# lupoglaz/DeepLocalProteinDocking

Hardware: AMD Instinct MI355X
Metric: pose correlations/sec (48ch x 64^3 pair, 6-degree SOI-sized generated rotation set) (higher is better)
Workload: dtype f32

## Files before the change

### deeplocalproteindocking_amd/csrc/dlpd_corr.hip

```cpp
#include <dlpd_platform.h>
#include "dlpd_fft.h"
#include "dlpd_internal.h"
#include "dlpd_trilinear.h"
#include "dlpd_k1.h"
#include "dlpd_k3.h"

#ifndef DLPD_K1CL_PAD
#define DLPD_K1CL_PAD 13
#endif
#ifndef DLPD_K1CL_PXOR
#define DLPD_K1CL_PXOR 0
#endif
#define DLPD_K1_UNROLL 2
DLPD_D float trilinear_fetch_quads(const float4* __restrict__ q, int L, float px, float py, float pz) {
  const float fx = floorf(px), fy = floorf(py), fz = floorf(pz);
  const int ix = (int)fx, iy = (int)fy, iz = (int)fz;
  const float ax = px - fx, ay = py - fy, az = pz - fz;
  const int hi = L - 1;
  const bool x0 = (ix >= 0) & (ix <= hi), x1 = (ix + 1 >= 0) & (ix + 1 <= hi);
  const bool y0 = (iy >= 0) & (iy <= hi), y1 = (iy + 1 >= 0) & (iy + 1 <= hi);
  const bool z0 = (iz >= 0) & (iz <= hi), z1 = (iz + 1 >= 0) & (iz + 1 <= hi);
  const float wx0 = x0 ? 1.f - ax : 0.f, wx1 = x1 ? ax : 0.f;
  const float wy0 = y0 ? 1.f - ay : 0.f, wy1 = y1 ? ay : 0.f;
  const float wz0 = z0 ? 1.f - az : 0.f, wz1 = z1 ? az : 0.f;
  const int cx0 = min(max(ix, 0), hi), cx1 = min(max(ix + 1, 0), hi);
  const int yb = min(max(iy, 0), hi - 1), zb = min(max(iz, 0), hi - 1);
  const int dy = iy - yb, dz = iz - zb;
  const int Q = L - 1;
  const float4 qa = q[((size_t)cx0 * Q + yb) * Q + zb];
  const float4 qb = q[((size_t)cx1 * Q + yb) * Q + zb];
  const float a_y0z0 = dy > 0 ? qa.z : qa.x, a_y0z1 = dy > 0 ? qa.w : qa.y;
  const float a_y1z0 = dy < 0 ? qa.x : qa.z, a_y1z1 = dy < 0 ? qa.y : qa.w;
  const float b_y0z0 = dy > 0 ? qb.z : qb.x, b_y0z1 = dy > 0 ? qb.w : qb.y;
  const float b_y1z0 = dy < 0 ? qb.x : qb.z, b_y1z1 = dy < 0 ? qb.y : qb.w;
  const float v000 = dz > 0 ? a_y0z1 : a_y0z0, v001 = dz < 0 ? a_y0z0 : a_y0z1;
  const float v010 = dz > 0 ? a_y1z1 : a_y1z0, v011 = dz < 0 ? a_y1z0 : a_y1z1;
  const float v100 = dz > 0 ? b_y0z1 : b_y0z0, v101 = dz < 0 ? b_y0z0 : b_y0z1;
  const float v110 = dz > 0 ? b_y1z1 : b_y1z0, v111 = dz < 0 ? b_y1z0 : b_y1z1;
  float acc = v000 * (wx0 * wy0 * wz0);
  acc += v001 * (wx0 * wy0 * wz1);
  acc += v010 * (wx0 * wy1 * wz0);
  acc += v011 * (wx0 * wy1 * wz1);
  acc += v100 * (wx1 * wy0 * wz0);
  acc += v101 * (wx1 * wy0 * wz1);
  acc += v110 * (wx1 * wy1 * wz0);
  acc += v111 * (wx1 * wy1 * wz1);
  return acc;
}

__global__ void __launch_bounds__(256) k_make_quads(const float* __restrict__ v, float4* __restrict__ q, int nvol, int L) {
  const int Q = L - 1;
  const size_t total = (size_t)nvol * L * Q * Q;
  for (size_t i = (size_t)blockIdx.x * blockDim.x + threadIdx.x; i < total; i += (size_t)gridDim.x * blockDim.x) {
    const int z = (int)(i % Q), y = (int)((i / Q) % Q);
    const size_t xv = i / ((size_t)Q * Q);
    const float* p = v + (xv * L + y) * L + z;
    q[i] = make_float4(p[0], p[1], p[L], p[L + 1]);
  }
}

__global__ void __launch_bounds__(256) k_rotate(const float* __restrict__ vol, const float* __restrict__ R,
                                                float* __restrict__ out, int B, int C, int L,
                                                long long vol_bstride, float c0) {
  const size_t L3 = (size_t)L * L * L;
  const size_t total = (size_t)B * C * L3;
  for (size_t i = (size_t)blockIdx.x * blockDim.x + threadIdx.x; i < total; i += (size_t)gridDim.x * blockDim.x) {
    const int z = (int)(i % L), y = (int)((i / L) % L), x = (int)((i / ((size_t)L * L)) % L);
    const int c = (int)((i / L3) % C), b = (int)(i / (L3 * C));
    const float* r = R + (size_t)b * 9;
    const float dx = x - c0, dy = y - c0, dz = z - c0;
    const float px = c0 + (r[0] * dx + r[3] * dy + r[6] * dz);
    const float py = c0 + (r[1] * dx + r[4] * dy + r[7] * dz);
    const float pz = c0 + (r[2] * dx + r[5] * dy + r[8] * dz);
    out[i] = trilinear_fetch(vol + (size_t)b * vol_bstride + (size_t)c * L3, L, px, py, pz);
  }
}

#ifdef DLPD_STAMPS
__device__ unsigned long long dlpd_stamps_k1[16];
extern "C" int dlpd_debug_read_stamps_k1(unsigned long long* host16) {
  if (hipMemcpyFromSymbol(host16, HIP_SYMBOL(dlpd_stamps_k1), 16 * sizeof(unsigned long long)) != hipSuccess) return 1;
  unsigned long long z[16] = {0};
  return hipMemcpyToSymbol(HIP_SYMBOL(dlpd_stamps_k1), z, sizeof(z)) == hipSuccess ? 0 : 1;
}
#endif
template <int N> __global__ void __launch_bounds__((N / 4) * FftPlan<N>::T)
k_rotate_zfft(const float* __restrict__ vol, const float* __restrict__ R, cplx* __restrict__ A,
              int CT, int nb, long long vol_bstride, int do_rotate, float c0, int CT_out, int c_base,
              int transposed, const float4* __restrict__ quads, int ext, const unsigned char* __restrict__ occ, int skip_empty) {
  constexpr int L = N / 2, NZ = N / 2 + 1, RS = N + 1, NP = L / 2;
  constexpr int T = FftPlan<N>::T, R1 = FftPlan<N>::R1, R2 = FftPlan<N>::R2;
  constexpr int NT = NP * T;
  __shared__ cplx S[NP * RS + N];
  cplx* tw = S + NP * RS;
  const int tid = threadIdx.x;
  const int bid = blockIdx.x, jj = bid >> 3;
  const int grp = (bid & 7) + 8 * (jj / L);
  if (grp >= CT * nb) return;
  const int c = grp % CT, b = grp / CT;
  if (do_rotate || !occ) init_twiddles<N>(tw, tid, NT);
  const int tr_flag = transposed;
  const int lane = tid & 63, wave = tid >> 6;
  (void)lane; (void)wave;
  DLPD_STAMP_DECL;
  const int x = jj % L;
  bool pencil_live = true;
  {
  const float* v = vol + (size_t)b * vol_bstride + (size_t)c * L * L * L;
  float* Sf = reinterpret_cast<float*>(S);
  if (do_rotate) {
    const float* r = R + (size_t)b * 9;
    const float r0 = r[tr_flag ? 3 : 0], r1 = r[tr_flag ? 4 : 1], r2 = r[tr_flag ? 5 : 2];
    const float r3 = r[tr_flag ? 0 : 3], r4 = r[tr_flag ? 1 : 4], r5 = r[tr_flag ? 2 : 5];
    const float r6 = r[6], r7 = r[7], r8 = r[8];
    const float dx = x - c0;
#pragma unroll DLPD_K1_UNROLL
    for (int s = tid; s < L * L; s += NT) {
      constexpr int TZ = 8, TYY = 64 / TZ;
      const int chunk = s >> 6, q = s & 63;
      const int y = (chunk / (L / TZ)) * TYY + q / TZ, z = (chunk % (L / TZ)) * TZ + q % TZ;
      const float dy = y - c0, dz = z - c0;
      const float px = c0 + (r0 * dx + r3 * dy + r6 * dz);
      const float py = c0 + (r1 * dx + r4 * dy + r7 * dz);
      const float pz = c0 + (r2 * dx + r5 * dy + r8 * dz);
      Sf[((y >> 1) * RS + z) * 2 + (y & 1)] =
          (max(x, max(y, z)) >= ext) ? 0.f
          : quads ? trilinear_fetch_quads(quads + (size_t)c * L * (L - 1) * (L - 1), L, px, py, pz)
                  : trilinear_fetch(v, L, px, py, pz);
    }
  } else {
    constexpr int NC = (L + 3) / 4;
    const unsigned char* ob = occ ? occ + ((size_t)b * NC + (x >> 2)) * NC * NC : nullptr;
    __shared__ unsigned char ocell[NC * NC];
    __shared__ int occ_any, yany[NC];
    if (ob) {
      if (tid == 0) occ_any = 0;
      if (tid < NC) yany[tid] = 0;
      __syncthreads();
      for (int i = tid; i < NC * NC; i += NT) {
        const unsigned char o = ob[i];
        ocell[i] = o;
        if (o) { occ_any = 1; yany[i / NC] = 1; }
      }
      __syncthreads();
      if (!occ_any) {
        if (skip_empty) return;
        cplx* a = A + ((size_t)b * CT_out + c_base + c) * NZ * L * L + (size_t)x * L;
        for (int s = tid; s < NP * NZ; s += NT)
          DLPD_STORE_STREAM(reinterpret_cast<float4*>(a + (size_t)(s / NP) * L * L + 2 * (s % NP)), make_float4(0.f, 0.f, 0.f, 0.f));
        return;
      }
      init_twiddles<N>(tw, tid, NT);
    }
    for (int s = tid; s < L * L; s += NT) {
      const int y = s / L, z = s % L;
      const bool zero = ob && !ocell[(y >> 2) * NC + (z >> 2)];
      Sf[((y >> 1) * RS + z) * 2 + (y & 1)] = zero ? 0.f : (tr_flag ? v[((size_t)y * L + x) * L + z] : v[((size_t)x * L + y) * L + z]);
    }
    pencil_live = !(ob && skip_empty) || yany[(tid % NP) >> 1];
  }
  DLPD_STAMP(0);
  __syncthreads();
  DLPD_STAMP(1);
  const int p = tid % NP, t = tid / NP;
  {
    FftPass<N, R1, 1, -1, T, L> ps;
    if (pencil_live) ps.load(S + p * RS, 1, t, tw);
    __syncthreads();
    if (pencil_live) ps.store(S + p * RS, 1, t);
    __syncthreads();
  }
  {
    FftPass<N, R2, R1, -1, T> ps;
    if (pencil_live) ps.load(S + p * RS, 1, t, tw);
    __syncthreads();
    if (pencil_live) ps.store(S + p * RS, 1, t);
    __syncthreads();
  }
  DLPD_STAMP(2);
  cplx* a = A + ((size_t)b * CT_out + c_base + c) * NZ * L * L + (size_t)x * L;
  for (int s = tid; s < NP * NZ; s += NT) {
    const int m = s % NP, k = s / NP;
    if (!pencil_live) continue;
    const cplx zk = S[m * RS + k];
    const cplx zn = S[m * RS + ((N - k) % N)];
    float4 o;
    o.x = 0.5f * (zk.x + zn.x);
    o.y = 0.5f * (zk.y - zn.y);
    o.z = 0.5f * (zk.y + zn.y);
    o.w = 0.5f * (zn.x - zk.x);
    DLPD_STORE_STREAM(reinterpret_cast<float4*>(a + (size_t)k * L * L + 2 * m), o);
  }
  DLPD_STAMP(3);
  }
  DLPD_STAMP_FLUSH(dlpd_stamps_k1, DLPD_STAMPS);
}

template <int N, bool OCC> __global__ void __launch_bounds__(K1ClCfg<N>::NP * FftPlan<N>::T)
k_rotate_zfft_cl(const float4* __restrict__ cl, const float* __restrict__ R, cplx* __restrict__ A,
                 int C, int nchunk, int vstride, int cstride, int nb, float c0, int CT_out, int c_base, int ext,
                 const unsigned char* __restrict__ occ, int skip_empty) {
  constexpr int L = N / 2, NZ = N / 2 + 1, NP = K1ClCfg<N>::NP, CC = K1ClCfg<N>::CC, YG = K1ClCfg<N>::YG, NPR = YG / 2;
  constexpr int LPV = CC / 4, SKEW = 16 / LPV;
  static_assert(CC * NPR == NP && L % YG == 0 && (NP * FftPlan<N>::T) % 64 == 0, "whole waves of pencils per block");
  constexpr int RS = N + DLPD_K1CL_PAD;
  constexpr int T = FftPlan<N>::T, R1 = FftPlan<N>::R1, R2 = FftPlan<N>::R2;
  constexpr int NT = NP * T;
  DLPD_DYN_SHARED(cplx, S);
  cplx* tw = S + NP * RS;
  const int tid = threadIdx.x;
  const int per = (L / YG) * nchunk;
  const int groups = nb * L, gper = (groups + 7) / 8;
  const int bid = blockIdx.x, seq = bid >> 3;
  const int g = (bid & 7) * gper + seq / per;
  if (seq / per >= gper || g >= groups) return;
#ifdef DLPD_K1_CHUNK_OUTER
  const int inner = seq % per, chunk = inner / (L / YG), yg = inner % (L / YG);
#else
  const int inner = seq % per, yg = inner / nchunk, chunk = inner % nchunk;
#endif
  const int b = g / L, x = g % L;
  constexpr int NC = (L + 3) / 4, YC = YG / 4;
  static_assert(YG % 4 == 0, "a block's rows are whole cells");
  __shared__ unsigned char occ_s[OCC ? YC * NC : 1];
  __shared__ int occ_any;
  if (OCC) {
    const unsigned char* ob = occ + (((size_t)b * NC + (x >> 2)) * NC + (yg * YG >> 2)) * NC;
    if (tid == 0) occ_any = 0;
    __syncthreads();
    if (tid < YC * NC) {
      const unsigned char o = ob[tid];
      occ_s[tid] = o;
      if (o) occ_any = 1;
    }
    __syncthreads();
    if (!occ_any) {
      if (skip_empty) return;
      for (int s = tid; s < NP * NZ; s += NT) {
        const int pm = s % NP, k = s / NP;
        const int c = chunk * CC + pm / NPR, m = pm % NPR;
        if (c < C)
          DLPD_STORE_STREAM(reinterpret_cast<float4*>(A + (((size_t)b * CT_out + c_base + c) * NZ + k) * L * L + (size_t)x * L +
                                                      yg * YG + 2 * m), make_float4(0.f, 0.f, 0.f, 0.f));
      }
      return;
    }
  }
  init_twiddles<N>(tw, tid, NT);
  {
    const K1ClRot rot = k1cl_load_rotation(R + (size_t)b * 9);
    for (int task = tid; task < NPR * L * LPV; task += NT) {
      const int q = task % LPV, z = (task / LPV) % L, m = (task / LPV) / L;
      const float4* src = cl + (size_t)chunk * cstride + q;
      float4 acc[2];
      if (OCC && !occ_s[((2 * m) >> 2) * NC + (z >> 2)])
        acc[0] = acc[1] = make_float4(0.f, 0.f, 0.f, 0.f);
      else
        k1cl_sample_rows(src, vstride, L, ext, c0, rot, x, yg * YG + 2 * m, z, acc);
      cplx* P = S + ((4 * q) * NPR + m) * RS + SKEW * q + z;
      P[0] = c_make(acc[0].x, acc[1].x);
      P[NPR * RS] = c_make(acc[0].y, acc[1].y);
      P[2 * NPR * RS] = c_make(acc[0].z, acc[1].z);
      P[3 * NPR * RS] = c_make(acc[0].w, acc[1].w);
    }
  }
  __syncthreads();
  const int p = (tid % NP) ^ DLPD_K1CL_PXOR, t = tid / NP;
  cplx* Sp = S + p * RS + SKEW * (p / (4 * NPR));
  {
    FftPass<N, R1, 1, -1, T, L> ps;
    ps.load(Sp, 1, t, tw);
    __syncthreads();
    ps.store(Sp, 1, t);
    __syncthreads();
  }
  {
    FftPass<N, R2, R1, -1, T> ps;
    ps.load(Sp, 1, t, tw);
    __syncthreads();
    ps.store(Sp, 1, t);
    __syncthreads();
  }
  for (int s = tid; s < NP * NZ; s += NT) {
    const int pm = s % NP, k = s / NP;
    const int c = chunk * CC + pm / NPR, m = pm % NPR;
    if (c < C) {
      const cplx* Z = S + pm * RS + SKEW * (pm / (4 * NPR));
      const cplx zk = Z[k];
      const cplx zn = Z[(N - k) % N];
      float4 o;
      o.x = 0.5f * (zk.x + zn.x);
      o.y = 0.5f * (zk.y - zn.y);
      o.z = 0.5f * (zk.y + zn.y);
      o.w = 0.5f * (zn.x - zk.x);
      cplx* a = A + (((size_t)b * CT_out + c_base + c) * NZ + k) * L * L + (size_t)x * L + yg * YG + 2 * m;
      DLPD_STORE_STREAM(reinterpret_cast<float4*>(a), o);
    }
  }
}

__global__ void __launch_bounds__(256) k_make_channels_last(const float* __restrict__ v, float4* __restrict__ cl, int C, int Cq, int L) {
  const size_t L3 = (size_t)L * L * L, total = L3 * Cq;
  for (size_t i = (size_t)blockIdx.x * blockDim.x + threadIdx.x; i < total; i += (size_t)gridDim.x * blockDim.x) {
    const int c4 = (int)(i % Cq);
    const size_t vox = i / Cq;
    float e[4];
#pragma unroll
    for (int j = 0; j < 4; j++) e[j] = (4 * c4 + j < C) ? v[(size_t)(4 * c4 + j) * L3 + vox] : 0.f;
    cl[i] = make_float4(e[0], e[1], e[2], e[3]);
  }
}

__global__ void __launch_bounds__(256) k_make_channel_chunks(const float* __restrict__ v, float4* __restrict__ out, int C, int CCq,
                                                             int nchunk, int L) {
  const size_t L3 = (size_t)L * L * L, total = L3 * CCq * nchunk;
  for (size_t i = (size_t)blockIdx.x * blockDim.x + threadIdx.x; i < total; i += (size_t)gridDim.x * blockDim.x) {
    const int q = (int)(i % CCq);
    const size_t vox = (i / CCq) % L3;
    const int c0 = 4 * ((int)(i / (CCq * L3)) * CCq + q);
    float e[4];
#pragma unroll
    for (int j = 0; j < 4; j++) e[j] = (c0 + j < C) ? v[(size_t)(c0 + j) * L3 + vox] : 0.f;
    out[i] = make_float4(e[0], e[1], e[2], e[3]);
  }
}

template <int N> static int launch_k1_cl(const float4* cl, const float* R, cplx* A, int C, int nb, float c0, hipStream_t st,
                                         int CT_out, int c_base, int ext = 0, const unsigned char* occ = nullptr, int skip_empty = 0,
                                         bool chunk_major = false) {
  constexpr int L = N / 2, RS = N + DLPD_K1CL_PAD, CCq = K1ClCfg<N>::CC / 4;
  const int Cq = ((C + DLPD_K1CL_CC - 1) / DLPD_K1CL_CC) * (DLPD_K1CL_CC / 4);
  const int nchunk = chunk_major ? (C + 4 * CCq - 1) / (4 * CCq) : Cq / CCq;
  const int vstride = chunk_major ? CCq : Cq, cstride = chunk_major ? L * L * L * CCq : CCq;
  const size_t shmem = (size_t)(K1ClCfg<N>::NP * RS + N) * sizeof(cplx);
  const int per = (L / K1ClCfg<N>::YG) * nchunk;
  const int gper = (nb * L + 7) / 8;
  dim3 grid((unsigned)(8 * gper * per)), block(K1ClCfg<N>::NP * FftPlan<N>::T);
  const int e = (ext > 0 && ext < L) ? ext : L;
  if (occ) {
    int rc = dlpd_set_max_dyn_shared((const void*)k_rotate_zfft_cl<N, true>, shmem);
    if (rc) return rc;
    DLPD_LAUNCH((k_rotate_zfft_cl<N, true>), grid, block, shmem, st, cl, R, A, C, nchunk, vstride, cstride, nb, c0, CT_out,
                c_base, e, occ, skip_empty);
  } else {
    int rc = dlpd_set_max_dyn_shared((const void*)k_rotate_zfft_cl<N, false>, shmem);
    if (rc) return rc;
    DLPD_LAUNCH((k_rotate_zfft_cl<N, false>), grid, block, shmem, st, cl, R, A, C, nchunk, vstride, cstride, nb, c0, CT_out,
                c_base, e, occ, 0);
  }
  return dlpd_check_launch();
}

__global__ void __launch_bounds__(256) k_rotated_occupancy(const unsigned char* __restrict__ occ_src, const float* __restrict__ R,
                                                           unsigned char* __restrict__ occ_out, int nb, int L, float c0) {
  const int nc = (L + 3) / 4, nc3 = nc * nc * nc;
  for (int i = blockIdx.x * blockDim.x + threadIdx.x; i < nb * nc3; i += gridDim.x * blockDim.x) {
    const int b = i / nc3, cell = i % nc3, cz = cell % nc, cy = (cell / nc) % nc, cx = cell / (nc * nc);
    const float* r = R + (size_t)b * 9;
    const float hx = 0.5f * (min(4 * cx + 3, L - 1) - 4 * cx), hy = 0.5f * (min(4 * cy + 3, L - 1) - 4 * cy),
                hz = 0.5f * (min(4 * cz + 3, L - 1) - 4 * cz);
    const float dx = 4 * cx + hx - c0, dy = 4 * cy + hy - c0, dz = 4 * cz + hz - c0;
    bool any = false;
    int lo[3], hi[3];
#pragma unroll
    for (int a = 0; a < 3; a++) {
      const float s = c0 + (r[a] * dx + r[3 + a] * dy + r[6 + a] * dz);
      const float e = fabsf(r[a]) * hx + fabsf(r[3 + a]) * hy + fabsf(r[6 + a]) * hz + 1e-3f * (1.f + fabsf(s));
      lo[a] = max((int)floorf(s - e), 0) >> 2;
      hi[a] = min((int)floorf(s + e) + 1, L - 1) >> 2;
    }
    for (int sx = lo[0]; sx <= hi[0]; sx++)
      for (int sy = lo[1]; sy <= hi[1]; sy++)
        for (int sz = lo[2]; sz <= hi[2]; sz++) any |= occ_src[(sx * nc + sy) * nc + sz] != 0;
    occ_out[i] = any ? 1 : 0;
  }
}
__global__ void __launch_bounds__(256) k_pencil_bits(const unsigned char* __restrict__ occ, unsigned* __restrict__ bits, int nb, int nc) {
  const int lane = threadIdx.x & 63, i = (blockIdx.x * blockDim.x + threadIdx.x) >> 6;
  bool any = false;
  if (i < nb * nc && lane < nc) {
    const unsigned char* o = occ + ((size_t)i * nc + lane) * nc;
    for (int cz = 0; cz < nc; cz++) any |= o[cz] != 0;
  }
  const unsigned long long m = __ballot(any);
  if (i < nb * nc && lane == 0) bits[i] = (unsigned)m;
}

template <int N, int MODE> struct K3Cfg { static constexpr int NT = 512, WC = 8, TY = 16; };
#ifndef DLPD_K3_80_NT
#define DLPD_K3_80_NT 640
#endif
template <int MODE> struct K3Cfg<80, MODE> { static constexpr int NT = (MODE == 0 ? 320 : DLPD_K3_80_NT), WC = 5, TY = 16; };
template <> struct K3Cfg<160, 0> { static constexpr int NT = 320, WC = 5, TY = 16; };
#ifndef DLPD_K3_160_NT
#define DLPD_K3_160_NT 640
#endif
template <> struct K3Cfg<160, 1> { static constexpr int NT = DLPD_K3_160_NT, WC = 5, TY = 8; };
template <> struct K3Cfg<160, 2> { static constexpr int NT = DLPD_K3_160_NT, WC = 5, TY = 8; };
#ifndef DLPD_K3_LAUNDER_160
#define DLPD_K3_LAUNDER_160 1
#endif
#ifdef DLPD_STAMPS
__device__ unsigned long long dlpd_stamps[16];
#endif
template <int N, int HP, int MODE> __global__ void __launch_bounds__((K3Cfg<N, MODE>::NT))
k_zifft_filter(const cplx* __restrict__ Bw, float* __restrict__ out, int CT, int C, int has_clash, int G,
               const float* __restrict__ W1t, const float* __restrict__ b1, const float* __restrict__ W2,
               float b2, int has_clip, float clip, float thr, K3Aux aux, K3Cand cd) {
  typedef K3Cfg<N, MODE> Cfg;
  typedef K3Lds<N, Cfg> Geo;
  constexpr int NZ = Geo::NZ, RS = Geo::RS, TY = Cfg::TY, NPAIR = Geo::NPAIR;
  constexpr int NT = Cfg::NT, WC = Cfg::WC;
  constexpr int CPW = Geo::CPW;
  constexpr int LPK = Geo::LPK;
  static_assert((NPAIR == 8 || NPAIR == 4) && WC * 64 <= NT, "one wave = 8 pencils x 8 threads");
  constexpr int EPT = (NPAIR * N) / NT > 0 ? (NPAIR * N) / NT : 1;
  constexpr int MSTEP = NT / N;
  static_assert((NPAIR * N) % NT == 0 || NPAIR * N < NT, "tile/thread mismatch");
  constexpr int RAWC = Geo::RAWC;
  DLPD_DYN_SHARED(cplx, S);
  cplx* tw = S + WC * 8 * RS;
  float4* raw = reinterpret_cast<float4*>(tw + N);
  const int tid = threadIdx.x, lane = tid & 63, wave = tid >> 6;
  const int y0 = blockIdx.x * TY, xo = blockIdx.y, b = blockIdx.z;

  constexpr int HPH = HP;
  float nrm[EPT * 2];
  float total[EPT * 2];
#pragma unroll
  for (int e = 0; e < EPT * 2; e++) { nrm[e] = 0.f; total[e] = b2; }
  const unsigned cand_tau = (MODE == 1 && cd.keys) ? *cd.tau : 0u;
  if (MODE == 1 && cd.keys && !cand_tau && tid == 0) cd.count[cd.nb + blockIdx.z] = 1u;
  const int zz = tid % N, m0 = tid / N;
  const bool owner = (NPAIR * N >= NT) || (m0 < NPAIR);
  const int tr = lane & 7, qr = lane >> 3;
  float4* rawg = raw + wave * CPW * RAWC;

  constexpr int NFULL = (N / 2) / LPK;
  static_assert(NZ * NPAIR == NFULL * 64 + NPAIR, "raw channel = NFULL full DMA instructions + one short one");
  auto issue_channel = [&](int cb) {
#pragma unroll
    for (int j = 0; j < CPW; j++) {
      const int g = wave * CPW + j;
      if (g < G && cb + g < CT) {
        const cplx* src = Bw + (((size_t)b * CT + cb + g) * NZ * N + xo) * N + y0;
        const cplx* lane_src = src + (size_t)(lane / NPAIR) * N * N + 2 * (lane % NPAIR);
        float4* rj = rawg + j * RAWC;
#pragma unroll
        for (int it = 0; it < NFULL; it++) DLPD_GLDS16(lane_src + (size_t)it * LPK * N * N, rj + it * 64);
        const int mt = lane % NPAIR;
        DLPD_GLDS16(src + (size_t)(N / 2) * N * N + 2 * mt, rj + NFULL * 64);
      }
    }
  };
  DLPD_STAMP_DECL;
  issue_channel(0);
  init_twiddles<N>(tw, tid, NT);
  constexpr int j0 = 0;
  float h[EPT * 2][HPH > 0 ? HPH : 1];
  if (MODE >= 1) {
    if (MODE == 1 && aux.C > 0 && aux.is_preact) {
      const int Na = aux.N;
      const size_t cstride = (size_t)Na * Na * Na;
      const float* ab = aux.p + (size_t)b * HP * cstride + ((size_t)(xo >> 1) * Na + (y0 >> 1)) * Na + (zz >> 1);
      if (owner) {
#pragma unroll
        for (int e = 0; e < EPT; e++)
#pragma unroll
          for (int j = 0; j < HP; j++) {
            const float v = ab[(size_t)j * cstride + (size_t)(m0 + e * MSTEP) * Na];
            h[2 * e][j] = v;
            h[2 * e + 1][j] = v;
          }
      }
    } else {
#pragma unroll
      for (int e = 0; e < EPT * 2; e++)
#pragma unroll
        for (int j = 0; j < HPH; j++) h[e][j] = b1[j0 + j];
    }
  }
  __syncthreads();

  for (int cbase = 0; cbase < CT; cbase += G) {
    const int gn = (CT - cbase) < G ? (CT - cbase) : G;
    if (wave * CPW < gn) {
      DLPD_WAIT_VMEM();
      DLPD_WAVE_SYNC();
      DLPD_STAMP(0);
#pragma unroll
      for (int j = 0; j < CPW; j++) {
        if (wave * CPW + j >= gn) break;
        int m, kq, lq = lane;
        if (N == 160 && DLPD_K3_LAUNDER_160) DLPD_OPAQUE(lq);
        if (NPAIR == 8) {
          m = (lq & 3) | (((lq >> 4) & 1) << 2);
          kq = ((lq >> 2) & 1) | (((lq >> 5) & 1) << 1) | (((lq >> 3) & 1) << 2);
        } else {
          m = lq % NPAIR;
          kq = lq / NPAIR;
        }
        const int rot = (NPAIR == 8) ? 2 * m : 0;
        const int slot = NPAIR * kq + m;
        cplx* P = S + (wave * 8 + j * NPAIR + m) * RS;
        const float4* rj = rawg + j * RAWC;
        constexpr int PCH = NFULL > 8 ? NFULL / 2 : NFULL;
        const float4 qh = rj[NFULL * 64 + (lane % NPAIR)];
#pragma unroll
        for (int it0 = 0; it0 < NFULL; it0 += PCH) {
          float4 q[PCH];
          int kk[PCH];
#pragma unroll
          for (int u = 0; u < PCH; u++) {
            const int it = (it0 + u + rot) % NFULL;
            kk[u] = it * LPK + kq;
            q[u] = rj[it * 64 + slot];
          }
#pragma unroll
          for (int u = 0; u < PCH; u++) {
            const int k = kk[u];
            const cplx lo = (k == 0) ? c_make(q[u].x, q[u].z) : c_make(q[u].x - q[u].w, q[u].y + q[u].z);
            const cplx hi = (k == 0) ? c_make(q[u].x, q[u].z) : c_make(q[u].x + q[u].w, q[u].z - q[u].y);
            P[pencil_in_pos<N>(k)] = lo;
            P[pencil_in_pos<N>((N - k) & (k == 0 ? 0 : ~0))] = hi;
          }
        }
        if (lane / NPAIR == 0) S[(wave * 8 + j * NPAIR + lane % NPAIR) * RS + pencil_in_pos<N>(N / 2)] = c_make(qh.x, qh.z);
      }
      DLPD_WAIT_LDS();
      DLPD_WAVE_SYNC();
    }
    DLPD_STAMP(1);
    issue_channel(cbase + G);
    DLPD_STAMP(2);
    if (wave * CPW < gn) {
      int tq = tr, qq = qr;
      if (N == 160 && DLPD_K3_LAUNDER_160) { DLPD_OPAQUE(tq); DLPD_OPAQUE(qq); }
      fft_wave_pencils<N, +1>(S, wave * 8, RS, qq, tq, tw);
    }
    DLPD_STAMP(3);
    DLPD_LDS_BARRIER();
    DLPD_STAMP(4);
    if (owner) {
      if (MODE == 0) {
        for (int g = 0; g < gn; g++) {
          const int c = cbase + g;
#pragma unroll
          for (int e = 0; e < EPT; e++) {
            const int m = m0 + e * MSTEP;
            const cplx val = S[(g * NPAIR + m) * RS + pencil_out_pos<N>(zz)];
            float v0 = val.x, v1 = val.y;
            if (has_clip && c < C) { v0 = DLPD_CLAMP(v0, clip); v1 = DLPD_CLAMP(v1, clip); }
            float* o = out + ((((size_t)b * CT + c) * N + xo) * N + y0 + 2 * m) * N + zz;
            o[0] = v0;
            o[N] = v1;
          }
        }
      } else {
        const int gs = (cbase + gn <= C) ? gn : (C - cbase > 0 ? C - cbase : 0);
        float wcur[HPH > 0 ? HPH : 1], wnxt[HPH > 0 ? HPH : 1];
        cplx vcur[EPT], vnxt[EPT];
        if (gs > 0) {
#pragma unroll
          for (int j = 0; j < HPH; j++) wcur[j] = W1t[(size_t)cbase * HP + j0 + j];
#pragma unroll
          for (int e = 0; e < EPT; e++) vcur[e] = S[(m0 + e * MSTEP) * RS + pencil_out_pos<N>(zz)];
        }
        for (int g = 0; g < gs; g++) {
          const int gn1 = (g + 1 < gs ? g + 1 : g);
#pragma unroll
          for (int j = 0; j < HPH; j++) wnxt[j] = W1t[(size_t)(cbase + gn1) * HP + j0 + j];
#pragma unroll
          for (int e = 0; e < EPT; e++) vnxt[e] = S[(gn1 * NPAIR + m0 + e * MSTEP) * RS + pencil_out_pos<N>(zz)];
          DLPD_SCHED_FENCE();
#pragma unroll
          for (int e = 0; e < EPT; e++) {
            float v0 = vcur[e].x, v1 = vcur[e].y;
            if (has_clip) { v0 = DLPD_CLAMP(v0, clip); v1 = DLPD_CLAMP(v1, clip); }
#pragma unroll
            for (int j = 0; j < HPH; j++) {
              h[2 * e][j] = fmaf(wcur[j], v0, h[2 * e][j]);
              h[2 * e + 1][j] = fmaf(wcur[j], v1, h[2 * e + 1][j]);
            }
          }
          DLPD_SCHED_FENCE();
#pragma unroll
          for (int j = 0; j < HPH; j++) wcur[j] = wnxt[j];
#pragma unroll
          for (int e = 0; e < EPT; e++) vcur[e] = vnxt[e];
        }
        if (has_clash && cbase + gn > C) {
          const int g = C - cbase;
#pragma unroll
          for (int e = 0; e < EPT; e++) {
            const cplx v = S[(g * NPAIR + m0 + e * MSTEP) * RS + pencil_out_pos<N>(zz)];
            nrm[2 * e] = v.x;
            nrm[2 * e + 1] = v.y;
          }
        }
      }
    }
    DLPD_STAMP(5);
    DLPD_LDS_BARRIER();
    DLPD_STAMP(6);
  }
  DLPD_STAMP_FLUSH(dlpd_stamps, DLPD_STAMPS);
  if (MODE == 1 && owner && aux.C > 0 && !aux.is_preact) {
    const int Na = aux.N;
    const float* ab = aux.p + (size_t)b * aux.C * Na * Na * Na + ((size_t)(xo >> 1) * Na + (y0 >> 1)) * Na + (zz >> 1);
    constexpr int CH = EPT > 2 ? 4 : 8;
    const size_t cstride = (size_t)Na * Na * Na;
    for (int cb = 0; cb < aux.C; cb += CH) {
      float av[CH][EPT];
#pragma unroll
      for (int k = 0; k < CH; k++)
#pragma unroll
        for (int e = 0; e < EPT; e++)
          av[k][e] = (cb + k < aux.C) ? ab[(size_t)(cb + k) * cstride + (size_t)(m0 + e * MSTEP) * Na] : 0.f;
#pragma unroll
      for (int k = 0; k < CH; k++) {
        if (cb + k < aux.C) {
          const float* w = W1t + (size_t)(C + cb + k) * HP + j0;
#pragma unroll
          for (int e = 0; e < EPT; e++) {
            const float v = av[k][e];
#pragma unroll
            for (int j = 0; j < HPH; j++) {
              h[2 * e][j] = fmaf(w[j], v, h[2 * e][j]);
              h[2 * e + 1][j] = fmaf(w[j], v, h[2 * e + 1][j]);
            }
          }
        }
      }
    }
  }
  if (MODE == 1 && owner) {
#pragma unroll
    for (int e = 0; e < EPT * 2; e++)
#pragma unroll
      for (int j = 0; j < HPH; j++) total[e] = fmaf(W2[j0 + j], fmaxf(h[e][j], 0.f), total[e]);
  }
// ... 655 lines not shown
```

### deeplocalproteindocking_amd/csrc/dlpd_k1.h

```cpp
#pragma once
#include <dlpd_platform.h>
#include "dlpd_fft.h"

#define DLPD_K1CL_CC 16
#ifndef DLPD_K1_YG160
#define DLPD_K1_YG160 8
#endif
#ifndef DLPD_K1_CC160
#define DLPD_K1_CC160 16
#endif
#ifndef DLPD_K1_YG128
#define DLPD_K1_YG128 16
#endif
template <int N> struct K1ClCfg {
  static constexpr int YG = (N == 128) ? DLPD_K1_YG128 : (N == 160 ? DLPD_K1_YG160 : 8), CC = (N == 160) ? DLPD_K1_CC160 : 128 / YG;
  static constexpr int NP = CC * (YG / 2);
};
struct K1ClRot { float r0, r1, r2, r3, r4, r5, r6, r7, r8; };
DLPD_D K1ClRot k1cl_load_rotation(const float* r) {
  K1ClRot o = {r[0], r[1], r[2], r[3], r[4], r[5], r[6], r[7], r[8]};
  return o;
}

DLPD_D void k1cl_sample_rows(const float4* __restrict__ src, int Cq, int L, int ext, float c0, const K1ClRot& r, int x, int yrow,
                             int z, float4 (&acc)[2]) {
  const float dx = x - c0, dz = z - c0;
  const int hi = L - 1;
#pragma unroll
      for (int u = 0; u < 2; u++) {
        const bool live = max(x, max(yrow + u, z)) < ext;
        const float dy = (yrow + u) - c0;
        const float px = c0 + (r.r0 * dx + r.r3 * dy + r.r6 * dz);
        const float py = c0 + (r.r1 * dx + r.r4 * dy + r.r7 * dz);
        const float pz = c0 + (r.r2 * dx + r.r5 * dy + r.r8 * dz);
        const float fx = floorf(px), fy = floorf(py), fz = floorf(pz);
        const int ix = (int)fx, iy = (int)fy, iz = (int)fz;
        const float ax = px - fx, ay = py - fy, az = pz - fz;
        const bool x0 = live & (ix >= 0) & (ix <= hi), x1 = live & (ix + 1 >= 0) & (ix + 1 <= hi);
        const bool y0 = (iy >= 0) & (iy <= hi), y1 = (iy + 1 >= 0) & (iy + 1 <= hi);
        const bool z0 = (iz >= 0) & (iz <= hi), z1 = (iz + 1 >= 0) & (iz + 1 <= hi);
        const float wx0 = x0 ? 1.f - ax : 0.f, wx1 = x1 ? ax : 0.f;
        const float wy0 = y0 ? 1.f - ay : 0.f, wy1 = y1 ? ay : 0.f;
        const float wz0 = z0 ? 1.f - az : 0.f, wz1 = z1 ? az : 0.f;
        const int cx0 = min(max(ix, 0), hi), cx1 = min(max(ix + 1, 0), hi);
        const int cy0 = min(max(iy, 0), hi), cy1 = min(max(iy + 1, 0), hi);
        const int cz0 = min(max(iz, 0), hi), cz1 = min(max(iz + 1, 0), hi);
        const float4 v000 = src[(size_t)((cx0 * L + cy0) * L + cz0) * Cq], v001 = src[(size_t)((cx0 * L + cy0) * L + cz1) * Cq];
        const float4 v010 = src[(size_t)((cx0 * L + cy1) * L + cz0) * Cq], v011 = src[(size_t)((cx0 * L + cy1) * L + cz1) * Cq];
        const float4 v100 = src[(size_t)((cx1 * L + cy0) * L + cz0) * Cq], v101 = src[(size_t)((cx1 * L + cy0) * L + cz1) * Cq];
        const float4 v110 = src[(size_t)((cx1 * L + cy1) * L + cz0) * Cq], v111 = src[(size_t)((cx1 * L + cy1) * L + cz1) * Cq];
        const float w000 = wx0 * wy0 * wz0, w001 = wx0 * wy0 * wz1, w010 = wx0 * wy1 * wz0, w011 = wx0 * wy1 * wz1;
        const float w100 = wx1 * wy0 * wz0, w101 = wx1 * wy0 * wz1, w110 = wx1 * wy1 * wz0, w111 = wx1 * wy1 * wz1;
#define DLPD_TRI(f)                                                                                               \
  {                                                                                                               \
    float a = v000.f * w000;                                                                                      \
    a += v001.f * w001;                                                                                           \
    a += v010.f * w010;                                                                                           \
    a += v011.f * w011;                                                                                           \
    a += v100.f * w100;                                                                                           \
    a += v101.f * w101;                                                                                           \
    a += v110.f * w110;                                                                                           \
    a += v111.f * w111;                                                                                           \
    acc[u].f = a;                                                                                                 \
  }
        DLPD_TRI(x) DLPD_TRI(y) DLPD_TRI(z) DLPD_TRI(w)
#undef DLPD_TRI
      }
}

int dlpd_k1_role_split(const float4* cl, const float* R, cplx* A, int C, int nb, float c0, hipStream_t st, int CT_out, int c_base,
                       int ext, int L);
```

### deeplocalproteindocking_amd/csrc/dlpd_platform.h

```cpp
#pragma once
#include <hip/hip_runtime.h>
#include <stdint.h>

#define DLPD_HD __host__ __device__ __forceinline__
#define DLPD_D __device__ __forceinline__
#define DLPD_LAUNCH_RAW(kern, grid, block, shmem, stream, ...) \
  hipLaunchKernelGGL(kern, grid, block, shmem, stream, __VA_ARGS__)
#define DLPD_DYN_SHARED(type, name) extern __shared__ __attribute__((aligned(16))) unsigned char name##_raw_[]; \
  type* name = reinterpret_cast<type*>(name##_raw_)

__device__ __forceinline__ void dlpd_glds16(const void* g, void* l) {
  const unsigned la =
      __builtin_amdgcn_readfirstlane((unsigned)(size_t)(__attribute__((address_space(3))) void*)l);
  asm volatile("s_mov_b32 m0, %0\n\ts_nop 0\n\tglobal_load_lds_dwordx4 %1, off nt" ::"s"(la), "v"(g) : "memory", "m0");
}
#define DLPD_GLDS16(g, l) dlpd_glds16((const void*)(g), (void*)(l))
__device__ __forceinline__ void dlpd_glds16_so(const void* base, unsigned voff, void* l) {
  const unsigned la =
      __builtin_amdgcn_readfirstlane((unsigned)(size_t)(__attribute__((address_space(3))) void*)l);
  asm volatile("s_mov_b32 m0, %0\n\ts_nop 0\n\tglobal_load_lds_dwordx4 %1, %2 nt" ::"s"(la), "v"(voff), "s"(base) : "memory", "m0");
}
#define DLPD_GLDS16_SO(base, voff, l) dlpd_glds16_so((const void*)(base), (unsigned)(voff), (void*)(l))
typedef unsigned dlpd_lds_t;
__device__ __forceinline__ dlpd_lds_t dlpd_lds_addr(void* l) {
  return __builtin_amdgcn_readfirstlane((unsigned)(size_t)(__attribute__((address_space(3))) void*)l);
}
__device__ __forceinline__ void dlpd_glds16_soa(const void* base, unsigned voff, dlpd_lds_t la) {
  asm volatile("s_mov_b32 m0, %0\n\ts_nop 0\n\tglobal_load_lds_dwordx4 %1, %2 nt" ::"s"(la), "v"(voff), "s"(base) : "memory", "m0");
}
#define DLPD_LDS_ADDR(p) dlpd_lds_addr((void*)(p))
#define DLPD_GLDS16_SOA(base, voff, la) dlpd_glds16_soa((const void*)(base), (unsigned)(voff), (la))
#define DLPD_LDS_BARRIER() asm volatile("s_waitcnt lgkmcnt(0)\n\ts_barrier" ::: "memory")
#define DLPD_WAIT_VMEM() asm volatile("s_waitcnt vmcnt(0)" ::: "memory")
#define DLPD_HAS_LDS_ADDRESS_SPACE 1
#define DLPD_SET_PRIO(n) __builtin_amdgcn_s_setprio(n)
#define DLPD_WAVE_SYNC() asm volatile("" ::: "memory")
#define DLPD_WAIT_LDS() asm volatile("s_waitcnt lgkmcnt(0)" ::: "memory")
struct __attribute__((packed, aligned(4))) dlpd_pair_t { float x, y; };
#define DLPD_PAIR dlpd_pair_t
__device__ __forceinline__ dlpd_pair_t dlpd_load_pair(const float* p) { return *reinterpret_cast<const dlpd_pair_t*>(p); }
typedef float dlpd_f4v __attribute__((ext_vector_type(4)));
__device__ __forceinline__ float4 dlpd_load_stream(const float4* p) {
  const dlpd_f4v v = __builtin_nontemporal_load(reinterpret_cast<const dlpd_f4v*>(p));
  return make_float4(v.x, v.y, v.z, v.w);
}
__device__ __forceinline__ void dlpd_store_stream(float4* p, float4 v) {
  const dlpd_f4v q = {v.x, v.y, v.z, v.w};
  __builtin_nontemporal_store(q, reinterpret_cast<dlpd_f4v*>(p));
}
__device__ __forceinline__ void dlpd_store_stream_c(float2* p, float2 v) {
  typedef float dlpd_f2s __attribute__((ext_vector_type(2)));
  const dlpd_f2s q = {v.x, v.y};
  __builtin_nontemporal_store(q, reinterpret_cast<dlpd_f2s*>(p));
}
__device__ __forceinline__ float2 dlpd_load_stream_c(const float2* p) {
  typedef float dlpd_f2s __attribute__((ext_vector_type(2)));
  const dlpd_f2s v = __builtin_nontemporal_load(reinterpret_cast<const dlpd_f2s*>(p));
  return make_float2(v.x, v.y);
}
#define DLPD_LOAD_STREAM(p) dlpd_load_stream(p)
#define DLPD_STORE_STREAM(p, v) dlpd_store_stream((p), (v))
#include <stdlib.h>
#define DLPD_CLAMP(v, c) __builtin_amdgcn_fmed3f((v), -(c), (c))
#define DLPD_SCHED_FENCE() __builtin_amdgcn_sched_barrier(0)
#define DLPD_OPAQUE_V(x) asm volatile("" : "+v"(x))
#define DLPD_UNIFORM(x) __builtin_amdgcn_readfirstlane(x)
#define DLPD_SINK_S(x) asm volatile("" ::"s"(x))
#define DLPD_SINK_V(x) asm volatile("" ::"v"(x))
#define DLPD_OPAQUE_S(x) asm volatile("" : "+s"(x))
#define DLPD_OPAQUE(x) asm volatile("" : "+v"(x))
typedef float dlpd_f2v __attribute__((ext_vector_type(2)));
__device__ __forceinline__ dlpd_f2v dlpd_f2_make(float a, float b) { dlpd_f2v r = {a, b}; return r; }
__device__ __forceinline__ dlpd_f2v dlpd_f2_splat(float a) { dlpd_f2v r = {a, a}; return r; }
__device__ __forceinline__ float dlpd_f2_get(dlpd_f2v v, int i) { return i ? v.y : v.x; }
__device__ __forceinline__ dlpd_f2v dlpd_pk_fma(dlpd_f2v a, dlpd_f2v b, dlpd_f2v c) { return __builtin_elementwise_fma(a, b, c); }

__device__ __forceinline__ void dlpd_lds_count(unsigned* table, unsigned bin, bool hit, int lane) {
  unsigned long long todo = __ballot(hit);
  unsigned mine = 0;
  while (todo) {
    const int first = __builtin_ctzll(todo);
    const unsigned fb = (unsigned)__builtin_amdgcn_readlane((int)bin, first);
    const unsigned long long same = __ballot(hit && bin == fb);
    if (lane == first) mine = (unsigned)__popcll(same);
    todo &= ~same;
  }
  if (mine) table[bin] += mine;
}

#ifndef DLPD_PK
#define DLPD_PK 1
#endif
#if DLPD_PK
#define DLPD_PKV(a) dlpd_f2_make((a).x, (a).y)
__device__ __forceinline__ float2 dlpd_pkf(dlpd_f2v v) { return make_float2(v.x, v.y); }
__device__ __forceinline__ float2 dlpd_c_add(float2 a, float2 b) { return dlpd_pkf(DLPD_PKV(a) + DLPD_PKV(b)); }
__device__ __forceinline__ float2 dlpd_c_sub(float2 a, float2 b) { return dlpd_pkf(DLPD_PKV(a) - DLPD_PKV(b)); }
__device__ __forceinline__ float2 dlpd_c_scale(float2 a, float s) { return dlpd_pkf(DLPD_PKV(a) * s); }
__device__ __forceinline__ float2 dlpd_c_axpy(float2 a, float s, float2 b) {
  return dlpd_pkf(__builtin_elementwise_fma(dlpd_f2_splat(s), DLPD_PKV(b), DLPD_PKV(a)));
}
__device__ __forceinline__ float2 dlpd_c_add_mi(float2 a, float2 b) {
  dlpd_f2v d;
  asm("v_pk_add_f32 %0, %1, %2 op_sel:[0,1] op_sel_hi:[1,0] neg_hi:[0,1]" : "=v"(d) : "v"(DLPD_PKV(a)), "v"(DLPD_PKV(b)));
  return dlpd_pkf(d);
}
__device__ __forceinline__ float2 dlpd_c_add_pi(float2 a, float2 b) {
  dlpd_f2v d;
  asm("v_pk_add_f32 %0, %1, %2 op_sel:[0,1] op_sel_hi:[1,0] neg_lo:[0,1]" : "=v"(d) : "v"(DLPD_PKV(a)), "v"(DLPD_PKV(b)));
  return dlpd_pkf(d);
}
__device__ __forceinline__ float2 dlpd_c_rotcs_m(float2 a, float c, float s) {
  const dlpd_f2v va = DLPD_PKV(a), t = va * c, vs = dlpd_f2_splat(s);
  dlpd_f2v d;
  asm("v_pk_fma_f32 %0, %1, %2, %3 op_sel:[1,0,0] op_sel_hi:[0,1,1] neg_hi:[1,0,0]" : "=v"(d) : "v"(va), "s"(vs), "v"(t));
  return dlpd_pkf(d);
}
__device__ __forceinline__ float2 dlpd_c_rotcs_p(float2 a, float c, float s) {
  const dlpd_f2v va = DLPD_PKV(a), t = va * c, vs = dlpd_f2_splat(s);
  dlpd_f2v d;
  asm("v_pk_fma_f32 %0, %1, %2, %3 op_sel:[1,0,0] op_sel_hi:[0,1,1] neg_lo:[1,0,0]" : "=v"(d) : "v"(va), "s"(vs), "v"(t));
  return dlpd_pkf(d);
}
__device__ __forceinline__ float2 dlpd_c_mul(float2 a, float2 w) {
  dlpd_f2v t, d;
  const dlpd_f2v va = DLPD_PKV(a), vw = DLPD_PKV(w);
  asm("v_pk_mul_f32 %0, %1, %2 op_sel:[1,1] op_sel_hi:[1,0] neg_lo:[0,1]" : "=v"(t) : "v"(va), "v"(vw));
  asm("v_pk_fma_f32 %0, %1, %2, %3 op_sel_hi:[0,1,1]" : "=v"(d) : "v"(va), "v"(vw), "v"(t));
  return dlpd_pkf(d);
}
__device__ __forceinline__ float2 dlpd_c_mulc(float2 a, float2 w) {
  dlpd_f2v t, d;
  const dlpd_f2v va = DLPD_PKV(a), vw = DLPD_PKV(w);
  asm("v_pk_mul_f32 %0, %1, %2 op_sel:[1,1] op_sel_hi:[1,0]" : "=v"(t) : "v"(va), "v"(vw));
  asm("v_pk_fma_f32 %0, %1, %2, %3 op_sel_hi:[0,1,1] neg_hi:[1,0,0]" : "=v"(d) : "v"(va), "v"(vw), "v"(t));
  return dlpd_pkf(d);
}
#endif

typedef float dlpd_acc4 __attribute__((ext_vector_type(4)));
__device__ __forceinline__ dlpd_acc4 dlpd_acc4_zero() { dlpd_acc4 z = {0.f, 0.f, 0.f, 0.f}; return z; }
__device__ __forceinline__ float dlpd_acc4_get(dlpd_acc4 v, int j) { return v[j]; }
__device__ __forceinline__ dlpd_acc4 dlpd_acc4_make(float a, float b, float c, float d) { dlpd_acc4 z = {a, b, c, d}; return z; }
#define DLPD_MFMA_16x16x4(a, b, acc) __builtin_amdgcn_mfma_f32_16x16x4f32((a), (b), (acc), 0, 0, 0)
typedef __bf16 dlpd_bf16x8 __attribute__((ext_vector_type(8)));
__device__ __forceinline__ dlpd_acc4 dlpd_mfma_16x16x32_bf16(float4 a, float4 b, dlpd_acc4 acc) {
  return __builtin_amdgcn_mfma_f32_16x16x32_bf16(__builtin_bit_cast(dlpd_bf16x8, a), __builtin_bit_cast(dlpd_bf16x8, b), acc, 0, 0, 0);
}
#define DLPD_MFMA_16x16x32_BF16(a, b, acc) dlpd_mfma_16x16x32_bf16((a), (b), (acc))
__device__ __forceinline__ unsigned dlpd_f2bf(float x) { return (unsigned)__builtin_bit_cast(unsigned short, (__bf16)x); }
__device__ __forceinline__ float dlpd_bf2f(unsigned h) { return __uint_as_float(h << 16); }
```

Measured before the change: 6.875 billion.

## Split trilinear z-pair gathers across lane pairs with DPP exchange in rotate kernel

Adds a ZP variant of the rotate+z-FFT kernel for N=128 with chunk-major layout. Each task now covers one z-corner of a row pair instead of both. A lane gathers its own corner plus the neighbour row's matching corner and swaps the second set with its quad partner through a DPP quad permute, which halves each lane's gather width and spreads global loads across more lanes. Loads for DEPTH tasks are issued before any are consumed, to give more memory-level parallelism. The cost is extra register pressure, scattered float-wide shared stores, and correctness that depends on the ownership logic at clamped z boundaries.

```diff
diff --git a/deeplocalproteindocking_amd/csrc/dlpd_corr.hip b/deeplocalproteindocking_amd/csrc/dlpd_corr.hip
--- a/deeplocalproteindocking_amd/csrc/dlpd_corr.hip
+++ b/deeplocalproteindocking_amd/csrc/dlpd_corr.hip
@@ -196,7 +196,7 @@
   DLPD_STAMP_FLUSH(dlpd_stamps_k1, DLPD_STAMPS);
 }
 
-template <int N, bool OCC> __global__ void __launch_bounds__(K1ClCfg<N>::NP * FftPlan<N>::T)
+template <int N, bool OCC, bool ZP = false> __global__ void __launch_bounds__(K1ClCfg<N>::NP * FftPlan<N>::T)
 k_rotate_zfft_cl(const float4* __restrict__ cl, const float* __restrict__ R, cplx* __restrict__ A,
                  int C, int nchunk, int vstride, int cstride, int nb, float c0, int CT_out, int c_base, int ext,
                  const unsigned char* __restrict__ occ, int skip_empty) {
@@ -249,19 +249,47 @@
   init_twiddles<N>(tw, tid, NT);
   {
     const K1ClRot rot = k1cl_load_rotation(R + (size_t)b * 9);
-    for (int task = tid; task < NPR * L * LPV; task += NT) {
-      const int q = task % LPV, z = (task / LPV) % L, m = (task / LPV) / L;
-      const float4* src = cl + (size_t)chunk * cstride + q;
-      float4 acc[2];
-      if (OCC && !occ_s[((2 * m) >> 2) * NC + (z >> 2)])
-        acc[0] = acc[1] = make_float4(0.f, 0.f, 0.f, 0.f);
-      else
-        k1cl_sample_rows(src, vstride, L, ext, c0, rot, x, yg * YG + 2 * m, z, acc);
-      cplx* P = S + ((4 * q) * NPR + m) * RS + SKEW * q + z;
-      P[0] = c_make(acc[0].x, acc[1].x);
-      P[NPR * RS] = c_make(acc[0].y, acc[1].y);
-      P[2 * NPR * RS] = c_make(acc[0].z, acc[1].z);
-      P[3 * NPR * RS] = c_make(acc[0].w, acc[1].w);
+    if constexpr (ZP) {
+      static_assert(LPV == 2 && (NPR * L * 4) % NT == 0 && L % 16 == 0, "whole waves of four-lane tasks, one row pair per wave");
+      constexpr int DEPTH = DLPD_K1_ZPAIR_DEPTH;
+      static_assert((NPR * L * 4) % (DEPTH * NT) == 0, "every lane has DEPTH tasks per round");
+      for (int task0 = tid; task0 < NPR * L * 4; task0 += DEPTH * NT) {
+        K1ClZpairTask tk[DEPTH];
+#pragma unroll
+        for (int i = 0; i < DEPTH; i++) {
+          const int task = task0 + i * NT;
+          const int q = task & 1, zc = (task >> 1) & 1, z = (task >> 2) % L, m = (task >> 2) / L;
+          const bool gather = !OCC || occ_s[((2 * m) >> 2) * NC + (z >> 2)];
+          k1cl_zpair_issue(tk[i], cl + (size_t)chunk * cstride + q, LPV, L, ext, c0, rot, x, yg * YG + 2 * m, z, zc, gather);
+        }
+        DLPD_SCHED_FENCE();
+#pragma unroll
+        for (int i = 0; i < DEPTH; i++) {
+          const int task = task0 + i * NT;
+          const int q = task & 1, zc = (task >> 1) & 1, z = (task >> 2) % L, m = (task >> 2) / L;
+          const float4 acc = k1cl_zpair_finish(tk[i]);
+          float* P = reinterpret_cast<float*>(S + ((4 * q) * NPR + m) * RS + SKEW * q + z) + zc;
+          P[0] = acc.x;
+          P[2 * NPR * RS] = acc.y;
+          P[4 * NPR * RS] = acc.z;
+          P[6 * NPR * RS] = acc.w;
+        }
+      }
+    } else {
+      for (int task = tid; task < NPR * L * LPV; task += NT) {
+        const int q = task % LPV, z = (task / LPV) % L, m = (task / LPV) / L;
+        const float4* src = cl + (size_t)chunk * cstride + q;
+        float4 acc[2];
+        if (OCC && !occ_s[((2 * m) >> 2) * NC + (z >> 2)])
+          acc[0] = acc[1] = make_float4(0.f, 0.f, 0.f, 0.f);
+        else
+          k1cl_sample_rows(src, vstride, L, ext, c0, rot, x, yg * YG + 2 * m, z, acc);
+        cplx* P = S + ((4 * q) * NPR + m) * RS + SKEW * q + z;
+        P[0] = c_make(acc[0].x, acc[1].x);
+        P[NPR * RS] = c_make(acc[0].y, acc[1].y);
+        P[2 * NPR * RS] = c_make(acc[0].z, acc[1].z);
+        P[3 * NPR * RS] = c_make(acc[0].w, acc[1].w);
+      }
     }
   }
   __syncthreads();
@@ -337,6 +365,20 @@
   const int gper = (nb * L + 7) / 8;
   dim3 grid((unsigned)(8 * gper * per)), block(K1ClCfg<N>::NP * FftPlan<N>::T);
   const int e = (ext > 0 && ext < L) ? ext : L;
+  if constexpr (K1ClZpair<N>::ON) {
+    if (chunk_major) {
+      int rc = occ ? dlpd_set_max_dyn_shared((const void*)k_rotate_zfft_cl<N, true, true>, shmem)
+                   : dlpd_set_max_dyn_shared((const void*)k_rotate_zfft_cl<N, false, true>, shmem);
+      if (rc) return rc;
+      if (occ)
+        DLPD_LAUNCH((k_rotate_zfft_cl<N, true, true>), grid, block, shmem, st, cl, R, A, C, nchunk, vstride, cstride, nb, c0, CT_out,
+                    c_base, e, occ, skip_empty);
+      else
+        DLPD_LAUNCH((k_rotate_zfft_cl<N, false, true>), grid, block, shmem, st, cl, R, A, C, nchunk, vstride, cstride, nb, c0, CT_out,
+                    c_base, e, occ, 0);
+      return dlpd_check_launch();
+    }
+  }
   if (occ) {
     int rc = dlpd_set_max_dyn_shared((const void*)k_rotate_zfft_cl<N, true>, shmem);
     if (rc) return rc;
diff --git a/deeplocalproteindocking_amd/csrc/dlpd_k1.h b/deeplocalproteindocking_amd/csrc/dlpd_k1.h
--- a/deeplocalproteindocking_amd/csrc/dlpd_k1.h
+++ b/deeplocalproteindocking_amd/csrc/dlpd_k1.h
@@ -68,5 +68,101 @@
       }
 }
 
+#ifndef DLPD_K1_ZPAIR
+#define DLPD_K1_ZPAIR 1
+#endif
+#ifndef DLPD_K1_ZPAIR_DEPTH
+#define DLPD_K1_ZPAIR_DEPTH 2
+#endif
+#if !defined(DLPD_HAS_QUAD_SWAP2)
+DLPD_D float4 dlpd_quad_swap2(float4 v) {
+  const float2 a = __shfl_xor(make_float2(v.x, v.y), 2), b = __shfl_xor(make_float2(v.z, v.w), 2);
+  return make_float4(a.x, a.y, b.x, b.y);
+}
+#endif
+template <int N> struct K1ClZpair {
+  static constexpr bool ON = DLPD_K1_ZPAIR && N == 128 && K1ClCfg<N>::CC == 8;
+};
+struct K1ClPos { float ax, ay, az; int ix, iy, iz; };
+DLPD_D K1ClPos k1cl_position(float c0, const K1ClRot& r, float dx, float dy, float dz) {
+  const float px = c0 + (r.r0 * dx + r.r3 * dy + r.r6 * dz);
+  const float py = c0 + (r.r1 * dx + r.r4 * dy + r.r7 * dz);
+  const float pz = c0 + (r.r2 * dx + r.r5 * dy + r.r8 * dz);
+  const float fx = floorf(px), fy = floorf(py), fz = floorf(pz);
+  K1ClPos o = {px - fx, py - fy, pz - fz, (int)fx, (int)fy, (int)fz};
+  return o;
+}
+struct K1ClZpairTask {
+  float4 keep[4], send[4];
+  float wx0, wx1, wy0, wy1, wz0, wz1;
+  bool own0, own1, gather;
+};
+DLPD_D void k1cl_zpair_issue(K1ClZpairTask& t, const float4* __restrict__ src, int Cq, int L, int ext, float c0, const K1ClRot& r,
+                             int x, int yrow, int z, int zc, bool gather) {
+  const float4 zero = make_float4(0.f, 0.f, 0.f, 0.f);
+  const int hi = L - 1;
+  float4 (&keep)[4] = t.keep, (&send)[4] = t.send;
+  float &wx0 = t.wx0, &wx1 = t.wx1, &wy0 = t.wy0, &wy1 = t.wy1, &wz0 = t.wz0, &wz1 = t.wz1;
+  bool &own0 = t.own0, &own1 = t.own1;
+#pragma unroll
+  for (int j = 0; j < 4; j++) keep[j] = send[j] = zero;
+  wx0 = wx1 = wy0 = wy1 = wz0 = wz1 = 0.f;
+  own0 = own1 = false;
+  t.gather = gather;
+  if (gather) {
+    const float dx = x - c0, dz = z - c0;
+    const bool live = max(x, max(yrow + zc, z)) < ext;
+    const K1ClPos k = k1cl_position(c0, r, dx, (yrow + zc) - c0, dz);
+    const bool x0 = live & (k.ix >= 0) & (k.ix <= hi), x1 = live & (k.ix + 1 >= 0) & (k.ix + 1 <= hi);
+    const bool y0 = (k.iy >= 0) & (k.iy <= hi), y1 = (k.iy + 1 >= 0) & (k.iy + 1 <= hi);
+    const bool z0 = (k.iz >= 0) & (k.iz <= hi), z1 = (k.iz + 1 >= 0) & (k.iz + 1 <= hi);
+    wx0 = x0 ? 1.f - k.ax : 0.f, wx1 = x1 ? k.ax : 0.f;
+    wy0 = y0 ? 1.f - k.ay : 0.f, wy1 = y1 ? k.ay : 0.f;
+    wz0 = z0 ? 1.f - k.az : 0.f, wz1 = z1 ? k.az : 0.f;
+    const int zb = min(max(k.iz, 0), hi - 1), d = k.iz - zb;
+    own0 = (zc != 0) == (d > 0);
+    own1 = (zc != 0) == (d >= 0);
+    const K1ClPos s = k1cl_position(c0, r, dx, (yrow + (zc ^ 1)) - c0, dz);
+    const int sb = min(max(s.iz, 0), hi - 1);
+    const int kx0 = min(max(k.ix, 0), hi) * L, kx1 = min(max(k.ix + 1, 0), hi) * L;
+    const int ky0 = min(max(k.iy, 0), hi), ky1 = min(max(k.iy + 1, 0), hi);
+    const int sx0 = min(max(s.ix, 0), hi) * L, sx1 = min(max(s.ix + 1, 0), hi) * L;
+    const int sy0 = min(max(s.iy, 0), hi), sy1 = min(max(s.iy + 1, 0), hi);
+    const int kz = zb + zc, sz = sb + zc;
+    keep[0] = src[(size_t)((kx0 + ky0) * L + kz) * Cq], keep[1] = src[(size_t)((kx0 + ky1) * L + kz) * Cq];
+    keep[2] = src[(size_t)((kx1 + ky0) * L + kz) * Cq], keep[3] = src[(size_t)((kx1 + ky1) * L + kz) * Cq];
+    send[0] = src[(size_t)((sx0 + sy0) * L + sz) * Cq], send[1] = src[(size_t)((sx0 + sy1) * L + sz) * Cq];
+    send[2] = src[(size_t)((sx1 + sy0) * L + sz) * Cq], send[3] = src[(size_t)((sx1 + sy1) * L + sz) * Cq];
+  }
+}
+DLPD_D float4 k1cl_zpair_finish(const K1ClZpairTask& t) {
+  const float4 (&keep)[4] = t.keep;
+  const float wx0 = t.wx0, wx1 = t.wx1, wy0 = t.wy0, wy1 = t.wy1, wz0 = t.wz0, wz1 = t.wz1;
+  const bool own0 = t.own0, own1 = t.own1;
+  float4 recv[4];
+#pragma unroll
+  for (int j = 0; j < 4; j++) recv[j] = dlpd_quad_swap2(t.send[j]);
+  if (!t.gather) return make_float4(0.f, 0.f, 0.f, 0.f);
+  const float w000 = wx0 * wy0 * wz0, w001 = wx0 * wy0 * wz1, w010 = wx0 * wy1 * wz0, w011 = wx0 * wy1 * wz1;
+  const float w100 = wx1 * wy0 * wz0, w101 = wx1 * wy0 * wz1, w110 = wx1 * wy1 * wz0, w111 = wx1 * wy1 * wz1;
+  float4 acc;
+#define DLPD_TRI(f)                                                                                               \
+  {                                                                                                               \
+    _Pragma("clang fp contract(on)")                                                                              \
+    const float p1 = (own1 ? keep[0].f : recv[0].f) * w001;                                                       \
+    float a = (own0 ? keep[0].f : recv[0].f) * w000 + p1;                                                         \
+    a += (own0 ? keep[1].f : recv[1].f) * w010;                                                                   \
+    a += (own1 ? keep[1].f : recv[1].f) * w011;                                                                   \
+    a += (own0 ? keep[2].f : recv[2].f) * w100;                                                                   \
+    a += (own1 ? keep[2].f : recv[2].f) * w101;                                                                   \
+    a += (own0 ? keep[3].f : recv[3].f) * w110;                                                                   \
+    a += (own1 ? keep[3].f : recv[3].f) * w111;                                                                   \
+    acc.f = a;                                                                                                    \
+  }
+  DLPD_TRI(x) DLPD_TRI(y) DLPD_TRI(z) DLPD_TRI(w)
+#undef DLPD_TRI
+  return acc;
+}
+
 int dlpd_k1_role_split(const float4* cl, const float* R, cplx* A, int C, int nb, float c0, hipStream_t st, int CT_out, int c_base,
                        int ext, int L);
diff --git a/deeplocalproteindocking_amd/csrc/dlpd_platform.h b/deeplocalproteindocking_amd/csrc/dlpd_platform.h
--- a/deeplocalproteindocking_amd/csrc/dlpd_platform.h
+++ b/deeplocalproteindocking_amd/csrc/dlpd_platform.h
@@ -75,6 +75,14 @@
 __device__ __forceinline__ float dlpd_f2_get(dlpd_f2v v, int i) { return i ? v.y : v.x; }
 __device__ __forceinline__ dlpd_f2v dlpd_pk_fma(dlpd_f2v a, dlpd_f2v b, dlpd_f2v c) { return __builtin_elementwise_fma(a, b, c); }
 
+__device__ __forceinline__ float dlpd_quad_swap2(float v) {
+  return __int_as_float(__builtin_amdgcn_mov_dpp(__float_as_int(v), 0x4E, 0xF, 0xF, true));
+}
+__device__ __forceinline__ float4 dlpd_quad_swap2(float4 v) {
+  return make_float4(dlpd_quad_swap2(v.x), dlpd_quad_swap2(v.y), dlpd_quad_swap2(v.z), dlpd_quad_swap2(v.w));
+}
+#define DLPD_HAS_QUAD_SWAP2 1
+
 __device__ __forceinline__ void dlpd_lds_count(unsigned* table, unsigned bin, bool hit, int lane) {
   unsigned long long todo = __ballot(hit);
   unsigned mine = 0;
```

Result: faster. 6.957 billion (median of 6 runs) (+1.2%).
